# maelaubert/VulkanSift

Measured on AMD Instinct MI355X. Metric: SIFT detect+match frames/sec (640x480, ~2k kp), higher is better.
Workload: dtype f32

## Files before the change

### include/vksift_hip.h

```cpp
#ifndef VKSIFT_HIP_H
#define VKSIFT_HIP_H

#include <stddef.h>
#include <stdint.h>

#ifdef __cplusplus
extern "C"
{
#endif

#define VKSIFT_HIP_MAX_TAPS 20
#define VKSIFT_HIP_MATCH_CHUNKS 32
#define VKSIFT_HIP_MATCH_SMALL_NA 1536u
#define VKSIFT_HIP_MATCH_SMALL_NB 4096u
#define VKSIFT_HIP_MATCH_SCRATCH_U32(na, nb) (2u * (size_t)(na) + (size_t)(nb) + 72u + (size_t)(na) * 16u * VKSIFT_HIP_MATCH_CHUNKS)
#define VKSIFT_HIP_ABI_VERSION 6u
#define VKSIFT_HIP_GATHER_SLOTS 512u
#define VKSIFT_HIP_MATCH_SLOTS 256u
#define VKSIFT_HIP_MATCH_PK_NB 32768u
#define VKSIFT_HIP_MAX_ORI 18
#define VKSIFT_HIP_MAX_OCTAVE_SIDE 16383u

  typedef void *vksift_hip_stream;
  typedef void *vksift_hip_graph;
  typedef void *vksift_hip_event;

  int vksift_hip_init(void);
  uint32_t vksift_hip_abi_version(void);
  int vksift_hip_device_count(void);
  int vksift_hip_device_name(int idx, char *out256);
  int vksift_hip_set_device(int idx);
  size_t vksift_hip_device_free_mem(void);
  void *vksift_hip_malloc(size_t bytes);
  void vksift_hip_free(void *p);
  void *vksift_hip_host_malloc(size_t bytes);
  void vksift_hip_host_free(void *p);
  int vksift_hip_host_register(void *p, size_t bytes);
  int vksift_hip_host_unregister(void *p);
  int vksift_hip_is_pinned(const void *p);
  vksift_hip_stream vksift_hip_stream_create(void);
  void vksift_hip_stream_destroy(vksift_hip_stream s);
  int vksift_hip_stream_sync(vksift_hip_stream s);
  int vksift_hip_stream_busy(vksift_hip_stream s);
  vksift_hip_event vksift_hip_event_create(void);
  void vksift_hip_event_destroy(vksift_hip_event e);
  int vksift_hip_event_record(vksift_hip_event e, vksift_hip_stream s);
  int vksift_hip_event_sync(vksift_hip_event e);
  int vksift_hip_event_busy(vksift_hip_event e);
  float vksift_hip_event_elapsed_ms(vksift_hip_event a, vksift_hip_event b);
  int vksift_hip_stream_wait_event(vksift_hip_stream s, vksift_hip_event e);
  int vksift_hip_capture_begin(vksift_hip_stream s);
  int vksift_hip_capture_end(vksift_hip_stream s, vksift_hip_graph *out);
  int vksift_hip_graph_launch(vksift_hip_graph g, vksift_hip_stream s);
  void vksift_hip_graph_destroy(vksift_hip_graph g);
  int vksift_hip_memcpy_h2d(void *dst, const void *src, size_t n, vksift_hip_stream s);
  int vksift_hip_memcpy_d2h(void *dst, const void *src, size_t n, vksift_hip_stream s);
  int vksift_hip_memcpy_d2d(void *dst, const void *src, size_t n, vksift_hip_stream s);
  int vksift_hip_memcpy2d_d2h(void *dst, size_t dpitch, const void *src, size_t spitch, size_t width_bytes, size_t height, vksift_hip_stream s);
  int vksift_hip_post_words(uint32_t *host_mapped_dst, const uint32_t *src, size_t n_words, vksift_hip_stream s);
  int vksift_hip_memset(void *dst, int value, size_t n, vksift_hip_stream s);
  const char *vksift_hip_error_string(int err);
  void vksift_hip_range_push(const char *name);
  void vksift_hip_range_pop(void);

  enum
  {
    VKSIFT_TUNE_WG_TARGET = 0,
    VKSIFT_TUNE_WIDE_MASK = 1,
    VKSIFT_TUNE_MULTI_MAX = 2,
    VKSIFT_TUNE_REFINE_PTR = 3,
    VKSIFT_TUNE_SCAN_FORM = 4,
    VKSIFT_TUNE_PAIR_FORM = 5,
    VKSIFT_TUNE_PYR_GATE = 6,
    VKSIFT_TUNE_DENSE_ROWS = 7,
    VKSIFT_TUNE_SEED_WG = 8,
    VKSIFT_TUNE_SCAN_BAND = 9,
    VKSIFT_TUNE_TAIL_MULTI = 10,
    VKSIFT_TUNE_ZERO_COPY = 11,
    VKSIFT_TUNE_MIN_MARCH = 12,
    VKSIFT_TUNE_COUNT = 16
  };
  int vksift_hip_tune(int knob, int value);
  int vksift_hip_tune_get(int knob);


  typedef struct
  {
    float *base;
    uint32_t w, h;
    uint32_t pitch;
    uint64_t img_stride;
    uint32_t fp16;
    uint32_t reverse;
  } vksift_hip_Plane;

  int vksift_hip_input_blit(const uint8_t *src, uint32_t sw, uint32_t sh, uint64_t src_img_stride, vksift_hip_Plane dst, uint32_t batch,
                            vksift_hip_stream s);

  int vksift_hip_blur(vksift_hip_Plane src, vksift_hip_Plane dst, const float *taps, uint32_t ntaps, uint32_t batch, vksift_hip_stream s);

  int vksift_hip_blur_pair(vksift_hip_Plane src, vksift_hip_Plane dst1, vksift_hip_Plane dst2, const float *taps1, uint32_t ntaps1, const float *taps2,
                           uint32_t ntaps2, uint32_t batch, vksift_hip_stream s);

  int vksift_hip_blur_form(vksift_hip_Plane src, vksift_hip_Plane dst, uint32_t ntaps, uint32_t batch);

  int vksift_hip_blur_multi(const vksift_hip_Plane *src, const vksift_hip_Plane *dst, uint32_t n, const float *taps, uint32_t ntaps, uint32_t batch,
                            vksift_hip_stream s);

  int vksift_hip_blur_downsample(vksift_hip_Plane src, vksift_hip_Plane dst, vksift_hip_Plane next, const float *taps, uint32_t ntaps, uint32_t batch,
                                 vksift_hip_stream s);

  int vksift_hip_seed_upsampled(const uint8_t *src, uint32_t sw, uint32_t sh, uint64_t src_img_stride, vksift_hip_Plane dst, const float *taps, uint32_t ntaps,
                                uint32_t batch, vksift_hip_stream s);

  int vksift_hip_seed_direct(const uint8_t *src, uint32_t sw, uint32_t sh, uint64_t src_img_stride, vksift_hip_Plane dst, const float *taps, uint32_t ntaps,
                             uint32_t batch, vksift_hip_stream s);

  int vksift_hip_downsample(vksift_hip_Plane src, vksift_hip_Plane dst, uint32_t batch, vksift_hip_stream s);

  int vksift_hip_octave_chain(const vksift_hip_Plane *layers, uint32_t n_oct, uint32_t n_layers, uint32_t S, const float *taps, const uint32_t *ntaps,
                              uint32_t batch, vksift_hip_stream s);

  int vksift_hip_dog_plane(const float *lo, const float *hi, uint32_t w, uint32_t h, uint32_t pitch, uint32_t fp16, float *out_dense, vksift_hip_stream s);

  typedef struct
  {
    float *gauss;
    uint32_t fp16;
    uint32_t w, h, pitch;
    uint64_t plane_stride;
    uint64_t img_stride;
    uint32_t S;
    int32_t octave_idx;
    float seed_sigma;
    float dog_threshold;
    float edge_limit;
    uint8_t *feats;
    uint64_t feat_img_stride;
    uint32_t cap;
    uint32_t *found;
    uint32_t found_img_stride;
    uint64_t *seg_mask;
    uint32_t *seg_off;
    uint64_t seg_img_stride;
    uint32_t *cand_xy;
    uint32_t *cand_flag;
    uint32_t *cand_n;
    uint64_t cand_img_stride;
    uint32_t cand_cap;
    float *ori_ang;
    uint32_t *ori_cnt;
    uint64_t ori_img_stride;
    uint32_t max_ori;
    uint32_t use_vlfeat;
    const float *desc_fp_tab;
    uint32_t desc_fp_tab_len;
    uint32_t scan_reverse;
    uint32_t masks_cleared;
    uint32_t sec_index;
  } vksift_hip_OctaveJob;

  typedef struct
// ... 62 lines not shown
```

### vulkansift_amd/csrc/hip/extrema.hip

```cpp
#include <hip/hip_runtime.h>
#include <type_traits>
#include <stdint.h>
#include <stdlib.h>

#include "../detmath.h"
#include "multi.h"
#include "vksift_hip.h"

namespace
{

struct DogView
{
  const float *base;
  int w, h, pitch;
  size_t plane;
  int S;
  int fp16;
};

template <bool F16>
__device__ __forceinline__ float ld(const DogView &d, int s, int x, int y)
{
  if (s < 0 || s > d.S + 1)
    return 0.f;
  if (F16)
  {
    const _Float16 *p = (const _Float16 *)d.base + (size_t)s * d.plane + (size_t)y * d.pitch + x;
    return (float)(_Float16)((float)p[d.plane] - (float)p[0]);
  }
  const float *p = d.base + (size_t)s * d.plane + (size_t)y * d.pitch + x;
  return p[d.plane] - p[0];
}

struct KpRecord
{
  float x, y, scale_x, scale_y;
  uint32_t scale_idx;
  int32_t octave_idx;
  float sigma, orientation, intensity;
};

template <bool F16>
__device__ bool refine_texel(const DogView &d, int x, int y, int s, float dog_threshold, float edge_limit, float seed_sigma, int octave_idx, KpRecord *kp)
{
  const int W = d.w, H = d.h, S = d.S;
  float oX = 0.f, oY = 0.f, oS = 0.f, gX = 0.f, gY = 0.f, gS = 0.f;
  int rx = x, ry = y, rs = s;
  for (int step = 0; step < 5; step++)
  {
    float vc = ld<F16>(d, rs, rx, ry);
    float sp = ld<F16>(d, rs + 1, rx, ry), sm = ld<F16>(d, rs - 1, rx, ry);
    float xp = ld<F16>(d, rs, rx + 1, ry), xm = ld<F16>(d, rs, rx - 1, ry);
    float yp = ld<F16>(d, rs, rx, ry + 1), ym = ld<F16>(d, rs, rx, ry - 1);
    gS = 0.5f * (sp - sm);
    gX = 0.5f * (xp - xm);
    gY = 0.5f * (yp - ym);
    float h11 = sp + sm - 2.f * vc;
    float h22 = xp + xm - 2.f * vc;
    float h33 = yp + ym - 2.f * vc;
    float h12 = 0.25f * (ld<F16>(d, rs + 1, rx + 1, ry) - ld<F16>(d, rs + 1, rx - 1, ry) - ld<F16>(d, rs - 1, rx + 1, ry) + ld<F16>(d, rs - 1, rx - 1, ry));
    float h13 = 0.25f * (ld<F16>(d, rs + 1, rx, ry + 1) - ld<F16>(d, rs + 1, rx, ry - 1) - ld<F16>(d, rs - 1, rx, ry + 1) + ld<F16>(d, rs - 1, rx, ry - 1));
    float h23 = 0.25f * (ld<F16>(d, rs, rx + 1, ry + 1) - ld<F16>(d, rs, rx + 1, ry - 1) - ld<F16>(d, rs, rx - 1, ry + 1) + ld<F16>(d, rs, rx - 1, ry - 1));

    float det = h11 * ((h22 * h33) - (h23 * h23)) - h12 * ((h12 * h33) - (h13 * h23)) + h13 * ((h12 * h23) - (h13 * h22));
    if (det == 0.0f)
      return false;
    float i11 = ((h22 * h33) - (h23 * h23)) / det;
    float i12 = -1.f * ((h12 * h33) - (h13 * h23)) / det;
    float i13 = ((h12 * h23) - (h13 * h22)) / det;
    float i22 = ((h11 * h33) - (h13 * h13)) / det;
    float i23 = -1.f * ((h11 * h23) - (h13 * h12)) / det;
    float i33 = ((h11 * h22) - (h12 * h12)) / det;
    oS = -i11 * gS - i12 * gX - i13 * gY;
    oX = -i12 * gS - i22 * gX - i23 * gY;
    oY = -i13 * gS - i23 * gX - i33 * gY;

    if (fabsf(oX) < 0.6f && fabsf(oY) < 0.6f && fabsf(oS) < 0.6f)
      break;
    else if (step < 4)
    {
      rx += ((oX >= 0.6f && rx < (W - 2)) ? 1 : 0) + ((oX <= -0.6f && rx > 1) ? -1 : 0);
      ry += ((oY >= 0.6f && ry < (H - 2)) ? 1 : 0) + ((oY <= -0.6f && ry > 1) ? -1 : 0);
      rs += ((oS >= 0.6f && rs < (S + 1)) ? 1 : 0) + ((oS <= -0.6f && rs > 1) ? -1 : 0);
    }
  }
  float sx = (float)rx + oX, sy = (float)ry + oY, ss = (float)rs + oS;
  float vc = ld<F16>(d, rs, rx, ry);
  float nv = vc + 0.5f * (gX * oX + gY * oY + gS * oS);
  if (!(fabsf(nv) > dog_threshold && fabsf(oX) < 1.5f && fabsf(oY) < 1.5f && fabsf(oS) < 1.5f && sx >= 0 && sx < (float)W && sy >= 0 && sy < (float)H &&
        ss >= 0 && ss <= (float)(S + 1)))
    return false;
  float e11 = ld<F16>(d, rs, rx + 1, ry) + ld<F16>(d, rs, rx - 1, ry) - 2.f * vc;
  float e22 = ld<F16>(d, rs, rx, ry + 1) + ld<F16>(d, rs, rx, ry - 1) - 2.f * vc;
  float e12 = 0.25f * (ld<F16>(d, rs, rx + 1, ry + 1) - ld<F16>(d, rs, rx + 1, ry - 1) - ld<F16>(d, rs, rx - 1, ry + 1) + ld<F16>(d, rs, rx - 1, ry - 1));
  float edgeness = ((e11 + e22) * (e11 + e22)) / ((e11 * e22) - (e12 * e12));
  if (!((edgeness < edge_limit) && (edgeness >= 0)))
    return false;

  float scale_factor = octave_idx >= 0 ? dm_pow2i(octave_idx) : 1.f / dm_pow2i(-octave_idx);
  kp->scale_x = sx;
  kp->scale_y = sy;
  kp->scale_idx = (uint32_t)roundf(ss);
  kp->octave_idx = octave_idx;
  kp->sigma = seed_sigma * dm_exp2f(ss / (float)S) * scale_factor;
  kp->orientation = 0.f;
  kp->intensity = nv;
  kp->x = sx * scale_factor;
  kp->y = sy * scale_factor;
  return true;
}

template <bool F16>
__device__ bool refine_texel_buf(const __amdgpu_buffer_rsrc_t rsrc, int W, int H, int pitch, unsigned plane, int S, int x, int y, int s, float dog_threshold,
                                 float edge_limit, float seed_sigma, int octave_idx, KpRecord *kp)
{
  constexpr unsigned EB = F16 ? 2u : 4u;
  const int pitch_b = pitch * (int)EB;
  const unsigned plane_b = plane * EB;
  auto tex = [&](unsigned base, int row_off) -> float {
    if (F16)
      return (float)__builtin_bit_cast(_Float16, (unsigned short)__builtin_amdgcn_raw_buffer_load_b16(rsrc, base, row_off, 0));
    return __uint_as_float(__builtin_amdgcn_raw_buffer_load_b32(rsrc, base, row_off, 0));
  };
  auto dog = [&](float hi, float lo) -> float { return F16 ? (float)(_Float16)(hi - lo) : hi - lo; };
  float oX = 0.f, oY = 0.f, oS = 0.f, gX = 0.f, gY = 0.f, gS = 0.f;
  float vc = 0.f, xp = 0.f, xm = 0.f, yp = 0.f, ym = 0.f, h23 = 0.f;
  int rx = x, ry = y, rs = s;
  for (int step = 0; step < 5; step++)
  {
    const unsigned b0 = ((unsigned)rs * plane + (unsigned)(ry - 1) * (unsigned)pitch + (unsigned)(rx - 1)) * EB;
    const unsigned bm = b0 - plane_b, b1 = b0 + plane_b, b2 = b1 + plane_b;
    float g0[3][3], g1[3][3];
#pragma unroll
    for (int j = 0; j < 3; j++)
#pragma unroll
      for (int i = 0; i < 3; i++)
      {
        g0[j][i] = tex(b0 + (unsigned)i * EB, j * pitch_b);
        g1[j][i] = tex(b1 + (unsigned)i * EB, j * pitch_b);
      }
    const float gm_c = tex(bm + EB, pitch_b), gm_xm = tex(bm, pitch_b), gm_xp = tex(bm + 2u * EB, pitch_b), gm_ym = tex(bm + EB, 0), gm_yp = tex(bm + EB, 2 * pitch_b);
    const float g2_c = tex(b2 + EB, pitch_b), g2_xm = tex(b2, pitch_b), g2_xp = tex(b2 + 2u * EB, pitch_b), g2_ym = tex(b2 + EB, 0), g2_yp = tex(b2 + EB, 2 * pitch_b);
    const bool up = rs + 1 <= S + 1;
    const float sp = up ? dog(g2_c, g1[1][1]) : 0.f, sm = dog(g0[1][1], gm_c);
    const float p_xp = up ? dog(g2_xp, g1[1][2]) : 0.f, p_xm = up ? dog(g2_xm, g1[1][0]) : 0.f;
    const float p_yp = up ? dog(g2_yp, g1[2][1]) : 0.f, p_ym = up ? dog(g2_ym, g1[0][1]) : 0.f;
    const float m_xp = dog(g0[1][2], gm_xp), m_xm = dog(g0[1][0], gm_xm), m_yp = dog(g0[2][1], gm_yp), m_ym = dog(g0[0][1], gm_ym);
    float d0[3][3];
#pragma unroll
    for (int j = 0; j < 3; j++)
#pragma unroll
      for (int i = 0; i < 3; i++)
        d0[j][i] = dog(g1[j][i], g0[j][i]);
    vc = d0[1][1];
    xp = d0[1][2], xm = d0[1][0], yp = d0[2][1], ym = d0[0][1];
    gS = 0.5f * (sp - sm);
    gX = 0.5f * (xp - xm);
    gY = 0.5f * (yp - ym);
    float h11 = sp + sm - 2.f * vc;
    float h22 = xp + xm - 2.f * vc;
    float h33 = yp + ym - 2.f * vc;
    float h12 = 0.25f * (p_xp - p_xm - m_xp + m_xm);
    float h13 = 0.25f * (p_yp - p_ym - m_yp + m_ym);
    h23 = 0.25f * (d0[2][2] - d0[0][2] - d0[2][0] + d0[0][0]);

    float det = h11 * ((h22 * h33) - (h23 * h23)) - h12 * ((h12 * h33) - (h13 * h23)) + h13 * ((h12 * h23) - (h13 * h22));
    if (det == 0.0f)
      return false;
    float i11 = ((h22 * h33) - (h23 * h23)) / det;
    float i12 = -1.f * ((h12 * h33) - (h13 * h23)) / det;
    float i13 = ((h12 * h23) - (h13 * h22)) / det;
    float i22 = ((h11 * h33) - (h13 * h13)) / det;
    float i23 = -1.f * ((h11 * h23) - (h13 * h12)) / det;
    float i33 = ((h11 * h22) - (h12 * h12)) / det;
    oS = -i11 * gS - i12 * gX - i13 * gY;
    oX = -i12 * gS - i22 * gX - i23 * gY;
    oY = -i13 * gS - i23 * gX - i33 * gY;

    if (fabsf(oX) < 0.6f && fabsf(oY) < 0.6f && fabsf(oS) < 0.6f)
      break;
    else if (step < 4)
    {
      rx += ((oX >= 0.6f && rx < (W - 2)) ? 1 : 0) + ((oX <= -0.6f && rx > 1) ? -1 : 0);
      ry += ((oY >= 0.6f && ry < (H - 2)) ? 1 : 0) + ((oY <= -0.6f && ry > 1) ? -1 : 0);
      rs += ((oS >= 0.6f && rs < (S + 1)) ? 1 : 0) + ((oS <= -0.6f && rs > 1) ? -1 : 0);
    }
  }
  float sx = (float)rx + oX, sy = (float)ry + oY, ss = (float)rs + oS;
  float nv = vc + 0.5f * (gX * oX + gY * oY + gS * oS);
  if (!(fabsf(nv) > dog_threshold && fabsf(oX) < 1.5f && fabsf(oY) < 1.5f && fabsf(oS) < 1.5f && sx >= 0 && sx < (float)W && sy >= 0 && sy < (float)H &&
        ss >= 0 && ss <= (float)(S + 1)))
    return false;
  float e11 = xp + xm - 2.f * vc;
  float e22 = yp + ym - 2.f * vc;
  float e12 = h23;
  float edgeness = ((e11 + e22) * (e11 + e22)) / ((e11 * e22) - (e12 * e12));
  if (!((edgeness < edge_limit) && (edgeness >= 0)))
    return false;

  float scale_factor = octave_idx >= 0 ? dm_pow2i(octave_idx) : 1.f / dm_pow2i(-octave_idx);
  kp->scale_x = sx;
  kp->scale_y = sy;
  kp->scale_idx = (uint32_t)roundf(ss);
  kp->octave_idx = octave_idx;
  kp->sigma = seed_sigma * dm_exp2f(ss / (float)S) * scale_factor;
  kp->orientation = 0.f;
  kp->intensity = nv;
  kp->x = sx * scale_factor;
  kp->y = sy * scale_factor;
  return true;
}

struct ExtremaArgs
{
  const float *gauss;
  int fp16;
  int w, h, pitch;
  uint64_t plane_stride, img_stride;
  int S, octave_idx;
  float seed_sigma, dog_threshold, edge_limit;
  uint64_t *seg_mask;
  uint32_t *seg_off;
  uint64_t seg_img_stride;
  int nseg;
  uint8_t *feats;
  uint64_t feat_img_stride;
  uint32_t cap;
  uint32_t *found;
  uint32_t found_img_stride;
  uint32_t *cand_xy;
  uint32_t *cand_flag;
  uint32_t *cand_n;
  uint64_t cand_img_stride;
  uint32_t cand_cap;
  int band;
  uint32_t nsegs;
  uint32_t nchunks;
  int scan_rev;
};

__device__ __forceinline__ float wave_shr1(float v, float edge)
{
  return __builtin_bit_cast(float, __builtin_amdgcn_update_dpp(__builtin_bit_cast(int, edge), __builtin_bit_cast(int, v), 0x138, 0xf, 0xf, false));
}
__device__ __forceinline__ float wave_shl1(float v, float edge)
{
  return __builtin_bit_cast(float, __builtin_amdgcn_update_dpp(__builtin_bit_cast(int, edge), __builtin_bit_cast(int, v), 0x130, 0xf, 0xf, false));
}

__device__ __forceinline__ float fmax2(float a, float b)
{
  float r;
  asm("v_max_f32 %0, %1, %2" : "=v"(r) : "v"(a), "v"(b));
  return r;
}
__device__ __forceinline__ float fmin2(float a, float b)
{
  float r;
  asm("v_min_f32 %0, %1, %2" : "=v"(r) : "v"(a), "v"(b));
  return r;
}
__device__ __forceinline__ float fmax3(float a, float b, float c)
{
  float r;
  asm("v_max3_f32 %0, %1, %2, %3" : "=v"(r) : "v"(a), "v"(b), "v"(c));
  return r;
}
__device__ __forceinline__ float fmin3(float a, float b, float c)
{
  float r;
  asm("v_min3_f32 %0, %1, %2, %3" : "=v"(r) : "v"(a), "v"(b), "v"(c));
  return r;
}

__device__ __forceinline__ unsigned long long spread32(unsigned long long x)
{
  x &= 0xFFFFFFFFull;
  x = (x | (x << 16)) & 0x0000FFFF0000FFFFull;
  x = (x | (x << 8)) & 0x00FF00FF00FF00FFull;
  x = (x | (x << 4)) & 0x0F0F0F0F0F0F0F0Full;
  x = (x | (x << 2)) & 0x3333333333333333ull;
  x = (x | (x << 1)) & 0x5555555555555555ull;
  return x;
}

typedef unsigned u32x2_t __attribute__((ext_vector_type(2)));
constexpr unsigned EXT_OOB = 0x80000000u;

template <int S, int NSLOT, bool F16>
__global__ void __launch_bounds__(256, 4) k_extrema_lean(Multi<ExtremaArgs> m, int strip_major)
{
  const VBlock vb = vblock(m);
// ... 192 lines not shown
  uint32_t *__restrict__ chunk_tot = a.cand_flag;
  const uint64_t chunk_img_stride = a.cand_img_stride;
  const uint32_t n = a.nsegs;
  const int lane = threadIdx.x & 63, wave = threadIdx.x >> 6;
  const uint32_t i0 = vb.x * SEG_CHUNK + 4u * threadIdx.x;
  uint32_t p[4];
#pragma unroll
  for (int k = 0; k < 4; k++)
    p[k] = i0 + k < n ? (uint32_t)__popcll(mask[i0 + k]) : 0u;
  const uint32_t tsum = p[0] + p[1] + p[2] + p[3];
  uint32_t incl = tsum;
#pragma unroll
  for (int dlt = 1; dlt < 64; dlt <<= 1)
  {
    uint32_t t = __shfl_up(incl, dlt, 64);
    if (lane >= dlt)
      incl += t;
  }
  if (lane == 63)
    wave_tot[wave] = incl;
  __syncthreads();
  uint32_t wave_base = 0, total = 0;
  for (int wv = 0; wv < 16; wv++)
  {
    if (wv < wave)
      wave_base += wave_tot[wv];
    total += wave_tot[wv];
  }
  uint32_t run = wave_base + incl - tsum;
#pragma unroll
  for (int k = 0; k < 4; k++)
  {
    if (i0 + k < n)
      off[i0 + k] = run;
    run += p[k];
  }
  if (threadIdx.x == 0)
    chunk_tot[(size_t)b * chunk_img_stride + vb.x] = total;
}


__global__ void __launch_bounds__(256) k_cand_list(Multi<ExtremaArgs> mu)
{
  const VBlock vb = vblock(mu);
  const ExtremaArgs &a = mu.oct[vb.o];
  const uint32_t seg = vb.x * 256 + threadIdx.x;
  const int b = (int)vb.y;
  const uint32_t *chunk_tot = a.cand_flag + (size_t)b * a.cand_img_stride;
  if (vb.x == 0 && threadIdx.x == 0)
  {
    uint32_t total = 0;
    for (uint32_t c = 0; c < a.nchunks; c++)
      total += chunk_tot[c];
    a.cand_n[b] = total;
    if (total == 0)
      a.found[(size_t)b * a.found_img_stride] = 0;
  }
  unsigned long long m = seg < a.nsegs ? a.seg_mask[seg + (size_t)b * a.seg_img_stride] : 0ull;
  if (__ballot(m != 0ull) == 0ull)
    return;
  uint32_t base = 0;
  for (uint32_t c = threadIdx.x & 63u, nc = (vb.x * 256u) / SEG_CHUNK; c < nc; c += 64u)
    base += chunk_tot[c];
#pragma unroll
  for (int dlt = 32; dlt >= 1; dlt >>= 1)
    base += __shfl_xor(base, dlt, 64);
  if (m == 0ull)
    return;
  uint32_t pos = a.seg_off[seg + (size_t)b * a.seg_img_stride] + base;
  const uint32_t segx = seg % (uint32_t)a.nseg;
  const uint32_t yy = (seg / (uint32_t)a.nseg) % (uint32_t)a.h;
  const uint32_t sz = seg / ((uint32_t)a.nseg * (uint32_t)a.h);
  uint32_t *out = a.cand_xy + (size_t)b * a.cand_img_stride;
  while (m)
  {
    const int bit = __ffsll((long long)m) - 1;
    m &= m - 1;
    if (pos < a.cand_cap)
      out[pos] = (segx * 64u + (uint32_t)bit) | (yy << 14) | ((sz + 1u) << 28);
    pos++;
  }
}

template <bool F16, bool BUF>
__global__ void __launch_bounds__(256) k_refine_flags(Multi<ExtremaArgs> m)
{
  __shared__ uint32_t s_cnt[4];
  const VBlock vb = vblock(m);
  const ExtremaArgs &a = m.oct[vb.o];
  const int b = (int)vb.x;
  uint32_t n = a.cand_n[b];
  n = n < a.cand_cap ? n : a.cand_cap;
  const uint32_t nch = (n + 255u) / 256u;
  DogView d{(const float *)((const uint8_t *)a.gauss + (size_t)b * a.img_stride * (a.fp16 ? 2u : 4u)), a.w, a.h, a.pitch, (size_t)a.plane_stride, a.S, a.fp16};
  const __amdgpu_buffer_rsrc_t rsrc =
      __builtin_amdgcn_make_buffer_rsrc((void *)d.base, 0, (int)((unsigned)(a.S + 3) * (unsigned)a.plane_stride * (F16 ? 2u : 4u)), 0x00020000);
  const uint32_t *xy = a.cand_xy + (size_t)b * a.cand_img_stride;
  uint32_t *flag = a.cand_flag + (size_t)b * a.cand_img_stride;
  uint32_t *chunk_sum = a.seg_off + (size_t)b * a.seg_img_stride;
  for (uint32_t chunk = vb.y; chunk < nch; chunk += vb.gy)
  {
    const uint32_t i = chunk * 256u + threadIdx.x;
    bool ok = false;
    if (i < n)
    {
      const uint32_t c = xy[i];
      KpRecord kp;
      const int cx = (int)(c & 0x3fffu), cy = (int)((c >> 14) & 0x3fffu), cs = (int)(c >> 28);
      ok = BUF ? refine_texel_buf<F16>(rsrc, a.w, a.h, a.pitch, (unsigned)a.plane_stride, a.S, cx, cy, cs, a.dog_threshold, a.edge_limit, a.seed_sigma, a.octave_idx, &kp)
               : refine_texel<F16>(d, cx, cy, cs, a.dog_threshold, a.edge_limit, a.seed_sigma, a.octave_idx, &kp);
      flag[i] = ok ? 1u : 0u;
    }
    const unsigned long long bal = __ballot(ok);
    if ((threadIdx.x & 63) == 0)
      s_cnt[threadIdx.x >> 6] = (uint32_t)__popcll(bal);
    __syncthreads();
    if (threadIdx.x == 0)
      chunk_sum[chunk] = s_cnt[0] + s_cnt[1] + s_cnt[2] + s_cnt[3];
    __syncthreads();
  }
}

template <bool F16, bool BUF>
__global__ void __launch_bounds__(256) k_cand_emit(Multi<ExtremaArgs> m)
{
  __shared__ uint32_t s_cnt[4];
  __shared__ uint32_t s_red[4];
  __shared__ uint32_t s_list[256];
  const VBlock vb = vblock(m);
  const ExtremaArgs &a = m.oct[vb.o];
  const int b = (int)vb.x;
  const int lane = threadIdx.x & 63, wave = threadIdx.x >> 6;
  uint32_t n = a.cand_n[b];
  n = n < a.cand_cap ? n : a.cand_cap;
  const uint32_t nch = (n + 255u) / 256u;
  DogView d{(const float *)((const uint8_t *)a.gauss + (size_t)b * a.img_stride * (a.fp16 ? 2u : 4u)), a.w, a.h, a.pitch, (size_t)a.plane_stride, a.S, a.fp16};
  const __amdgpu_buffer_rsrc_t rsrc =
      __builtin_amdgcn_make_buffer_rsrc((void *)d.base, 0, (int)((unsigned)(a.S + 3) * (unsigned)a.plane_stride * (F16 ? 2u : 4u)), 0x00020000);
  const uint32_t *xy = a.cand_xy + (size_t)b * a.cand_img_stride;
  const uint32_t *flag = a.cand_flag + (size_t)b * a.cand_img_stride;
  const uint32_t *chunk_sum = a.seg_off + (size_t)b * a.seg_img_stride;
  for (uint32_t chunk = vb.y; chunk < nch; chunk += vb.gy)
  {
    uint32_t part = 0;
    for (uint32_t c = threadIdx.x; c < chunk; c += 256u)
      part += chunk_sum[c];
#pragma unroll
    for (int dlt = 32; dlt >= 1; dlt >>= 1)
      part += __shfl_xor(part, dlt, 64);
    const uint32_t i = chunk * 256u + threadIdx.x;
    const bool v = i < n && flag[i] != 0u;
    const unsigned long long bal = __ballot(v);
    if (lane == 0)
      s_cnt[wave] = (uint32_t)__popcll(bal), s_red[wave] = part;
    __syncthreads();
    const uint32_t cbase = s_red[0] + s_red[1] + s_red[2] + s_red[3];
    uint32_t rank = (uint32_t)__popcll(bal & ((1ull << lane) - 1ull));
    for (int wv = 0; wv < wave; wv++)
      rank += s_cnt[wv];
    const uint32_t total = s_cnt[0] + s_cnt[1] + s_cnt[2] + s_cnt[3];
    if (v)
      s_list[rank] = xy[i];
    __syncthreads();
    const uint32_t idx = cbase + threadIdx.x;
    if (chunk + 1u == nch && threadIdx.x == 0)
      a.found[(size_t)b * a.found_img_stride] = cbase + total;
    if (threadIdx.x < total && idx < a.cap)
    {
      const uint32_t c = s_list[threadIdx.x];
      KpRecord kp;
      const int cx = (int)(c & 0x3fffu), cy = (int)((c >> 14) & 0x3fffu), cs = (int)(c >> 28);
      if (BUF)
        refine_texel_buf<F16>(rsrc, a.w, a.h, a.pitch, (unsigned)a.plane_stride, a.S, cx, cy, cs, a.dog_threshold, a.edge_limit, a.seed_sigma, a.octave_idx, &kp);
      else
        refine_texel<F16>(d, cx, cy, cs, a.dog_threshold, a.edge_limit, a.seed_sigma, a.octave_idx, &kp);
      uint32_t *rec = (uint32_t *)(a.feats + (size_t)b * a.feat_img_stride + (size_t)idx * 164);
      rec[0] = __float_as_uint(kp.x);
      rec[1] = __float_as_uint(kp.y);
      rec[2] = __float_as_uint(kp.scale_x);
      rec[3] = __float_as_uint(kp.scale_y);
      rec[4] = kp.scale_idx;
      rec[5] = (uint32_t)kp.octave_idx;
      rec[6] = __float_as_uint(kp.sigma);
      rec[7] = __float_as_uint(kp.orientation);
      rec[8] = __float_as_uint(kp.intensity);
    }
    __syncthreads();
  }
}

}

static int make_extrema_args(const vksift_hip_OctaveJob *job, ExtremaArgs *out)
{
  if (job->w > VKSIFT_HIP_MAX_OCTAVE_SIDE || job->h > VKSIFT_HIP_MAX_OCTAVE_SIDE || job->S > 14u)
    return (int)hipErrorInvalidValue;
  ExtremaArgs a;
  a.gauss = job->gauss;
  a.fp16 = (int)job->fp16;
  a.w = (int)job->w, a.h = (int)job->h, a.pitch = (int)job->pitch;
  a.plane_stride = job->plane_stride, a.img_stride = job->img_stride;
  a.S = (int)job->S, a.octave_idx = job->octave_idx;
  a.seed_sigma = job->seed_sigma, a.dog_threshold = job->dog_threshold, a.edge_limit = job->edge_limit;
  a.seg_mask = job->seg_mask, a.seg_off = job->seg_off, a.seg_img_stride = job->seg_img_stride;
  a.nseg = (int)((job->w + 63) / 64);
  a.feats = job->feats, a.feat_img_stride = job->feat_img_stride, a.cap = job->cap;
  a.found = job->found, a.found_img_stride = job->found_img_stride;
  a.cand_xy = job->cand_xy, a.cand_flag = job->cand_flag, a.cand_n = job->cand_n;
  a.cand_img_stride = job->cand_img_stride, a.cand_cap = job->cand_cap;
  a.scan_rev = (int)job->scan_reverse;
  a.band = job->h > 256u ? 48 : 16;
  if (vksift_hip_tune_get(VKSIFT_TUNE_SCAN_BAND) > 0 && job->h > 256u)
    a.band = vksift_hip_tune_get(VKSIFT_TUNE_SCAN_BAND);
  a.nsegs = job->S * job->h * (uint32_t)a.nseg;
  a.nchunks = (a.nsegs + SEG_CHUNK - 1u) / SEG_CHUNK;
  if (job->seg_img_stride != a.nsegs || a.nchunks > a.cand_cap)
    return (int)hipErrorInvalidValue;
  *out = a;
  return 0;
}

static int clear_masks(const ExtremaArgs *args, uint32_t n, uint32_t batch, hipStream_t hs)
{
  for (uint32_t i = 0; i < n;)
  {
    uint32_t j = i + 1;
    size_t bytes = sizeof(uint64_t) * (size_t)args[i].nsegs * batch;
    while (j < n && (const uint8_t *)args[j].seg_mask == (const uint8_t *)args[i].seg_mask + bytes)
      bytes += sizeof(uint64_t) * (size_t)args[j].nsegs * batch, j++;
    const hipError_t me = hipMemsetAsync(args[i].seg_mask, 0, bytes, hs);
    if (me != hipSuccess)
      return (int)me;
    i = j;
  }
  return 0;
}

static int extract_run(const vksift_hip_OctaveJob *jobs, uint32_t n, uint32_t batch, hipStream_t hs, hipEvent_t scan_done)
{
  ExtremaArgs args[MULTI_MAX];
  for (uint32_t i = 0; i < n; i++)
  {
    const int e = make_extrema_args(&jobs[i], &args[i]);
    if (e)
      return e;
  }
  const bool f16 = args[0].fp16 != 0;
  const int S = args[0].S;
  {
    uint64_t waves = 0;
    for (uint32_t i = 0; i < n; i++)
      waves += (uint64_t)batch * ((args[i].w + 127) / 128) * ((args[i].h + args[i].band - 1) / args[i].band);
    if (waves < 2048u && vksift_hip_tune_get(VKSIFT_TUNE_SCAN_BAND) <= 0)
      for (uint32_t i = 0; i < n; i++)
        args[i].band = 16;
  }

  bool cleared = true;
  for (uint32_t i = 0; i < n; i++)
    cleared = cleared && jobs[i].masks_cleared != 0;
  if (!cleared)
  {
    const int me = clear_masks(args, n, batch, hs);
    if (me)
      return me;
  }
  const int sm = 3;
  for (uint32_t i = 0; i < n; i++)
    if ((uint64_t)jobs[i].pitch * jobs[i].h * (f16 ? 2u : 4u) >= 0x80000000ull)
      return (int)hipErrorInvalidValue;

#define VKSIFT_MULTI(M, GX, GY, GZ)                              \
  Multi<ExtremaArgs> M;                                           \
  M.n = 0;                                                        \
  for (uint32_t i = 0; i < n; i++)                                \
  {                                                               \
    const ExtremaArgs &a = args[i];                               \
    (void)a;                                                      \
    if (!multi_add(M, args[i], (GX), (GY), (GZ)))                 \
      return (int)hipErrorInvalidValue;                           \
  }
  {
    VKSIFT_MULTI(ms, (uint32_t)(a.nseg + 1) / 2u, ((a.h + a.band - 1) / a.band + 3u) / 4u, batch)
    const dim3 sgrid(ms.start[ms.n]);
    switch (S)
    {
#define VKSIFT_CASE(N)                                                                \
  case N:                                                                             \
    if (f16)                                                                          \
      hipLaunchKernelGGL((k_extrema_lean<N, 5, true>), sgrid, dim3(256), 0, hs, ms, sm);  \
    else                                                                              \
      hipLaunchKernelGGL((k_extrema_lean<N, 4, false>), sgrid, dim3(256), 0, hs, ms, sm); \
    break;
      VKSIFT_CASE(1) VKSIFT_CASE(2) VKSIFT_CASE(3) VKSIFT_CASE(4) VKSIFT_CASE(5) VKSIFT_CASE(6) VKSIFT_CASE(7) VKSIFT_CASE(8) VKSIFT_CASE(9)
      VKSIFT_CASE(10) VKSIFT_CASE(11) VKSIFT_CASE(12) VKSIFT_CASE(13)
#undef VKSIFT_CASE
    default:
      return (int)hipErrorInvalidValue;
    }
  }
  if (scan_done)
    (void)hipEventRecord(scan_done, hs);
  {
    VKSIFT_MULTI(m2, a.nchunks, batch, 1u)
    hipLaunchKernelGGL(k_segment_scan, dim3(m2.start[m2.n]), dim3(1024), 0, hs, m2);
  }
  {
    VKSIFT_MULTI(m3, (a.nsegs + 255u) / 256u, batch, 1u)
    hipLaunchKernelGGL(k_cand_list, dim3(m3.start[m3.n]), dim3(256), 0, hs, m3);
  }
  const uint32_t rcap = 65536u / batch < 16u ? 16u : (65536u / batch > 512u ? 512u : 65536u / batch);
#define VKSIFT_REFINE_CHUNKS(a) (((uint64_t)(a).S * (uint32_t)(a).w * (uint32_t)(a).h / 4u + 64u + 255u) / 256u)
  VKSIFT_MULTI(mr, batch, VKSIFT_REFINE_CHUNKS(a) > rcap ? rcap : (uint32_t)VKSIFT_REFINE_CHUNKS(a), 1u)
#undef VKSIFT_REFINE_CHUNKS
  const dim3 rgrid(mr.start[mr.n]);
  bool buf = vksift_hip_tune_get(VKSIFT_TUNE_REFINE_PTR) == 0;
  for (uint32_t i = 0; i < n; i++)
    buf = buf && (uint64_t)(args[i].S + 3) * args[i].plane_stride * (f16 ? 2u : 4u) < 0x7FFF0000ull;
  if (f16 && buf)
    hipLaunchKernelGGL((k_refine_flags<true, true>), rgrid, dim3(256), 0, hs, mr);
  else if (f16)
    hipLaunchKernelGGL((k_refine_flags<true, false>), rgrid, dim3(256), 0, hs, mr);
  else if (buf)
    hipLaunchKernelGGL((k_refine_flags<false, true>), rgrid, dim3(256), 0, hs, mr);
  else
    hipLaunchKernelGGL((k_refine_flags<false, false>), rgrid, dim3(256), 0, hs, mr);
  if (f16 && buf)
    hipLaunchKernelGGL((k_cand_emit<true, true>), rgrid, dim3(256), 0, hs, mr);
  else if (f16)
    hipLaunchKernelGGL((k_cand_emit<true, false>), rgrid, dim3(256), 0, hs, mr);
  else if (buf)
    hipLaunchKernelGGL((k_cand_emit<false, true>), rgrid, dim3(256), 0, hs, mr);
  else
    hipLaunchKernelGGL((k_cand_emit<false, false>), rgrid, dim3(256), 0, hs, mr);
#undef VKSIFT_MULTI
  return (int)hipGetLastError();
}

extern "C" int vksift_hip_extract_keypoints_multi(const vksift_hip_OctaveJob *jobs, uint32_t n_jobs, uint32_t batch, vksift_hip_stream s,
                                                  vksift_hip_event scan_done)
{
  if (n_jobs == 0 || batch == 0)
    return 0;
  for (uint32_t i0 = 0; i0 < n_jobs;)
  {
    uint32_t i1 = i0 + 1;
    while (i1 < n_jobs && i1 - i0 < multi_run_max() && jobs[i1].S == jobs[i0].S && jobs[i1].fp16 == jobs[i0].fp16)
      i1++;
    const int e = extract_run(jobs + i0, i1 - i0, batch, (hipStream_t)s, i1 == n_jobs ? (hipEvent_t)scan_done : nullptr);
    if (e)
      return e;
    i0 = i1;
  }
  return 0;
}

extern "C" int vksift_hip_clear_segment_masks(const vksift_hip_OctaveJob *jobs, uint32_t n_jobs, uint32_t batch, vksift_hip_stream s)
{
  if (n_jobs == 0 || batch == 0)
    return 0;
  if (n_jobs > 16)
    return (int)hipErrorInvalidValue;
  ExtremaArgs args[16];
  for (uint32_t i = 0; i < n_jobs; i++)
  {
    const int e = make_extrema_args(&jobs[i], &args[i]);
    if (e)
      return e;
  }
  return clear_masks(args, n_jobs, batch, (hipStream_t)s);
}

extern "C" int vksift_hip_extract_keypoints(const vksift_hip_OctaveJob *job, uint32_t batch, vksift_hip_stream s, vksift_hip_event scan_done)
{
  return vksift_hip_extract_keypoints_multi(job, 1, batch, s, scan_done);
}
```

Before: 25140.

## Refine keypoint candidates once and stash results in candidate buffers

Replaces the refine-flags plus emit pair, which ran the subpixel refinement twice per accepted candidate, with a single refinement pass. That pass writes the refined core values (position, scale, response) compactly into the candidate xy/flag buffers for chunks with few accepted points, and a move kernel then turns them into full records. Chunks with more accepted points than the cap fall back to flagging and re-refining. The old path stays selectable through a new tune knob, and the change adds per-chunk stash layout logic and a different grid cap for the move kernel.

New measurement: 25210 (median of 6 runs). No clear change (+0.3%).

```diff
diff --git a/include/vksift_hip.h b/include/vksift_hip.h
--- a/include/vksift_hip.h
+++ b/include/vksift_hip.h
@@ -78,6 +78,7 @@
     VKSIFT_TUNE_TAIL_MULTI = 10,
     VKSIFT_TUNE_ZERO_COPY = 11,
     VKSIFT_TUNE_MIN_MARCH = 12,
+    VKSIFT_TUNE_EXTRACT_FORM = 13,
     VKSIFT_TUNE_COUNT = 16
   };
   int vksift_hip_tune(int knob, int value);
diff --git a/vulkansift_amd/csrc/hip/extrema.hip b/vulkansift_amd/csrc/hip/extrema.hip
--- a/vulkansift_amd/csrc/hip/extrema.hip
+++ b/vulkansift_amd/csrc/hip/extrema.hip
@@ -41,8 +41,27 @@
   float sigma, orientation, intensity;
 };
 
+struct KpCore
+{
+  float sx, sy, ss, nv;
+};
+
+__device__ __forceinline__ void finish_record(const KpCore &c, int S, float seed_sigma, int octave_idx, KpRecord *kp)
+{
+  float scale_factor = octave_idx >= 0 ? dm_pow2i(octave_idx) : 1.f / dm_pow2i(-octave_idx);
+  kp->scale_x = c.sx;
+  kp->scale_y = c.sy;
+  kp->scale_idx = (uint32_t)roundf(c.ss);
+  kp->octave_idx = octave_idx;
+  kp->sigma = seed_sigma * dm_exp2f(c.ss / (float)S) * scale_factor;
+  kp->orientation = 0.f;
+  kp->intensity = c.nv;
+  kp->x = c.sx * scale_factor;
+  kp->y = c.sy * scale_factor;
+}
+
 template <bool F16>
-__device__ bool refine_texel(const DogView &d, int x, int y, int s, float dog_threshold, float edge_limit, float seed_sigma, int octave_idx, KpRecord *kp)
+__device__ bool refine_texel(const DogView &d, int x, int y, int s, float dog_threshold, float edge_limit, KpCore *kp)
 {
   const int W = d.w, H = d.h, S = d.S;
   float oX = 0.f, oY = 0.f, oS = 0.f, gX = 0.f, gY = 0.f, gS = 0.f;
@@ -98,22 +117,13 @@
   if (!((edgeness < edge_limit) && (edgeness >= 0)))
     return false;
 
-  float scale_factor = octave_idx >= 0 ? dm_pow2i(octave_idx) : 1.f / dm_pow2i(-octave_idx);
-  kp->scale_x = sx;
-  kp->scale_y = sy;
-  kp->scale_idx = (uint32_t)roundf(ss);
-  kp->octave_idx = octave_idx;
-  kp->sigma = seed_sigma * dm_exp2f(ss / (float)S) * scale_factor;
-  kp->orientation = 0.f;
-  kp->intensity = nv;
-  kp->x = sx * scale_factor;
-  kp->y = sy * scale_factor;
+  kp->sx = sx, kp->sy = sy, kp->ss = ss, kp->nv = nv;
   return true;
 }
 
 template <bool F16>
 __device__ bool refine_texel_buf(const __amdgpu_buffer_rsrc_t rsrc, int W, int H, int pitch, unsigned plane, int S, int x, int y, int s, float dog_threshold,
-                                 float edge_limit, float seed_sigma, int octave_idx, KpRecord *kp)
+                                 float edge_limit, KpCore *kp)
 {
   constexpr unsigned EB = F16 ? 2u : 4u;
   const int pitch_b = pitch * (int)EB;
@@ -199,16 +209,7 @@
   if (!((edgeness < edge_limit) && (edgeness >= 0)))
     return false;
 
-  float scale_factor = octave_idx >= 0 ? dm_pow2i(octave_idx) : 1.f / dm_pow2i(-octave_idx);
-  kp->scale_x = sx;
-  kp->scale_y = sy;
-  kp->scale_idx = (uint32_t)roundf(ss);
-  kp->octave_idx = octave_idx;
-  kp->sigma = seed_sigma * dm_exp2f(ss / (float)S) * scale_factor;
-  kp->orientation = 0.f;
-  kp->intensity = nv;
-  kp->x = sx * scale_factor;
-  kp->y = sy * scale_factor;
+  kp->sx = sx, kp->sy = sy, kp->ss = ss, kp->nv = nv;
   return true;
 }
 
@@ -567,6 +568,22 @@
   }
 }
 
+__device__ __forceinline__ void store_record(const ExtremaArgs &a, int b, uint32_t idx, const KpCore &kc)
+{
+  KpRecord kp;
+  finish_record(kc, a.S, a.seed_sigma, a.octave_idx, &kp);
+  uint32_t *rec = (uint32_t *)(a.feats + (size_t)b * a.feat_img_stride + (size_t)idx * 164);
+  rec[0] = __float_as_uint(kp.x);
+  rec[1] = __float_as_uint(kp.y);
+  rec[2] = __float_as_uint(kp.scale_x);
+  rec[3] = __float_as_uint(kp.scale_y);
+  rec[4] = kp.scale_idx;
+  rec[5] = (uint32_t)kp.octave_idx;
+  rec[6] = __float_as_uint(kp.sigma);
+  rec[7] = __float_as_uint(kp.orientation);
+  rec[8] = __float_as_uint(kp.intensity);
+}
+
 template <bool F16, bool BUF>
 __global__ void __launch_bounds__(256) k_refine_flags(Multi<ExtremaArgs> m)
 {
@@ -590,10 +607,10 @@
     if (i < n)
     {
       const uint32_t c = xy[i];
-      KpRecord kp;
+      KpCore kc;
       const int cx = (int)(c & 0x3fffu), cy = (int)((c >> 14) & 0x3fffu), cs = (int)(c >> 28);
-      ok = BUF ? refine_texel_buf<F16>(rsrc, a.w, a.h, a.pitch, (unsigned)a.plane_stride, a.S, cx, cy, cs, a.dog_threshold, a.edge_limit, a.seed_sigma, a.octave_idx, &kp)
-               : refine_texel<F16>(d, cx, cy, cs, a.dog_threshold, a.edge_limit, a.seed_sigma, a.octave_idx, &kp);
+      ok = BUF ? refine_texel_buf<F16>(rsrc, a.w, a.h, a.pitch, (unsigned)a.plane_stride, a.S, cx, cy, cs, a.dog_threshold, a.edge_limit, &kc)
+               : refine_texel<F16>(d, cx, cy, cs, a.dog_threshold, a.edge_limit, &kc);
       flag[i] = ok ? 1u : 0u;
     }
     const unsigned long long bal = __ballot(ok);
@@ -653,22 +670,146 @@
     if (threadIdx.x < total && idx < a.cap)
     {
       const uint32_t c = s_list[threadIdx.x];
-      KpRecord kp;
+      KpCore kc;
       const int cx = (int)(c & 0x3fffu), cy = (int)((c >> 14) & 0x3fffu), cs = (int)(c >> 28);
       if (BUF)
-        refine_texel_buf<F16>(rsrc, a.w, a.h, a.pitch, (unsigned)a.plane_stride, a.S, cx, cy, cs, a.dog_threshold, a.edge_limit, a.seed_sigma, a.octave_idx, &kp);
+        refine_texel_buf<F16>(rsrc, a.w, a.h, a.pitch, (unsigned)a.plane_stride, a.S, cx, cy, cs, a.dog_threshold, a.edge_limit, &kc);
       else
-        refine_texel<F16>(d, cx, cy, cs, a.dog_threshold, a.edge_limit, a.seed_sigma, a.octave_idx, &kp);
-      uint32_t *rec = (uint32_t *)(a.feats + (size_t)b * a.feat_img_stride + (size_t)idx * 164);
-      rec[0] = __float_as_uint(kp.x);
-      rec[1] = __float_as_uint(kp.y);
-      rec[2] = __float_as_uint(kp.scale_x);
-      rec[3] = __float_as_uint(kp.scale_y);
-      rec[4] = kp.scale_idx;
-      rec[5] = (uint32_t)kp.octave_idx;
-      rec[6] = __float_as_uint(kp.sigma);
-      rec[7] = __float_as_uint(kp.orientation);
-      rec[8] = __float_as_uint(kp.intensity);
+        refine_texel<F16>(d, cx, cy, cs, a.dog_threshold, a.edge_limit, &kc);
+      store_record(a, b, idx, kc);
+    }
+    __syncthreads();
+  }
+}
+
+constexpr uint32_t REC_CHUNK_CAP = 128;
+
+__device__ __forceinline__ bool chunk_is_compact(uint32_t chunk, uint32_t accepted, uint32_t rec_cap, uint32_t cand_cap)
+{
+  return accepted <= rec_cap && (uint64_t)chunk * 256u + 256u <= (uint64_t)cand_cap;
+}
+
+template <bool F16, bool BUF>
+__global__ void __launch_bounds__(256) k_refine_once(Multi<ExtremaArgs> m, uint32_t rec_cap)
+{
+  __shared__ uint32_t s_cnt[4];
+  const VBlock vb = vblock(m);
+  const ExtremaArgs &a = m.oct[vb.o];
+  const int b = (int)vb.x;
+  const int lane = threadIdx.x & 63, wave = threadIdx.x >> 6;
+  uint32_t n = a.cand_n[b];
+  n = n < a.cand_cap ? n : a.cand_cap;
+  const uint32_t nch = (n + 255u) / 256u;
+  DogView d{(const float *)((const uint8_t *)a.gauss + (size_t)b * a.img_stride * (a.fp16 ? 2u : 4u)), a.w, a.h, a.pitch, (size_t)a.plane_stride, a.S, a.fp16};
+  const __amdgpu_buffer_rsrc_t rsrc =
+      __builtin_amdgcn_make_buffer_rsrc((void *)d.base, 0, (int)((unsigned)(a.S + 3) * (unsigned)a.plane_stride * (F16 ? 2u : 4u)), 0x00020000);
+  uint32_t *xy = a.cand_xy + (size_t)b * a.cand_img_stride;
+  uint32_t *flag = a.cand_flag + (size_t)b * a.cand_img_stride;
+  uint32_t *chunk_sum = a.seg_off + (size_t)b * a.seg_img_stride;
+  for (uint32_t chunk = vb.y; chunk < nch; chunk += vb.gy)
+  {
+    const uint32_t i = chunk * 256u + threadIdx.x;
+    bool ok = false;
+    KpCore kc{0.f, 0.f, 0.f, 0.f};
+    if (i < n)
+    {
+      const uint32_t c = xy[i];
+      const int cx = (int)(c & 0x3fffu), cy = (int)((c >> 14) & 0x3fffu), cs = (int)(c >> 28);
+      ok = BUF ? refine_texel_buf<F16>(rsrc, a.w, a.h, a.pitch, (unsigned)a.plane_stride, a.S, cx, cy, cs, a.dog_threshold, a.edge_limit, &kc)
+               : refine_texel<F16>(d, cx, cy, cs, a.dog_threshold, a.edge_limit, &kc);
+    }
+    const unsigned long long bal = __ballot(ok);
+    if (lane == 0)
+      s_cnt[wave] = (uint32_t)__popcll(bal);
+    __syncthreads();
+    uint32_t rank = (uint32_t)__popcll(bal & ((1ull << lane) - 1ull));
+    for (int wv = 0; wv < wave; wv++)
+      rank += s_cnt[wv];
+    const uint32_t total = s_cnt[0] + s_cnt[1] + s_cnt[2] + s_cnt[3];
+    if (chunk_is_compact(chunk, total, rec_cap, a.cand_cap))
+    {
+      if (ok)
+      {
+        uint32_t *r0 = xy + (size_t)chunk * 256u + rank, *r1 = flag + (size_t)chunk * 256u + rank;
+        r0[0] = __float_as_uint(kc.sx), r0[REC_CHUNK_CAP] = __float_as_uint(kc.sy);
+        r1[0] = __float_as_uint(kc.ss), r1[REC_CHUNK_CAP] = __float_as_uint(kc.nv);
+      }
+    }
+    else if (i < n)
+      flag[i] = ok ? 1u : 0u;
+    if (threadIdx.x == 0)
+      chunk_sum[chunk] = total;
+    __syncthreads();
+  }
+}
+
+template <bool F16, bool BUF>
+__global__ void __launch_bounds__(256) k_cand_move(Multi<ExtremaArgs> m, uint32_t rec_cap)
+{
+  __shared__ uint32_t s_cnt[4];
+  __shared__ uint32_t s_red[4];
+  __shared__ uint32_t s_list[256];
+  const VBlock vb = vblock(m);
+  const ExtremaArgs &a = m.oct[vb.o];
+  const int b = (int)vb.x;
+  const int lane = threadIdx.x & 63, wave = threadIdx.x >> 6;
+  uint32_t n = a.cand_n[b];
+  n = n < a.cand_cap ? n : a.cand_cap;
+  const uint32_t nch = (n + 255u) / 256u;
+  const uint32_t *xy = a.cand_xy + (size_t)b * a.cand_img_stride;
+  const uint32_t *flag = a.cand_flag + (size_t)b * a.cand_img_stride;
+  const uint32_t *chunk_sum = a.seg_off + (size_t)b * a.seg_img_stride;
+  for (uint32_t chunk = vb.y; chunk < nch; chunk += vb.gy)
+  {
+    uint32_t part = 0;
+    for (uint32_t c = threadIdx.x; c < chunk; c += 256u)
+      part += chunk_sum[c];
+#pragma unroll
+    for (int dlt = 32; dlt >= 1; dlt >>= 1)
+      part += __shfl_xor(part, dlt, 64);
+    const uint32_t total = chunk_sum[chunk];
+    const bool compact = chunk_is_compact(chunk, total, rec_cap, a.cand_cap);
+    const uint32_t i = chunk * 256u + threadIdx.x;
+    const bool v = !compact && i < n && flag[i] != 0u;
+    const unsigned long long bal = __ballot(v);
+    if (lane == 0)
+      s_cnt[wave] = (uint32_t)__popcll(bal), s_red[wave] = part;
+    __syncthreads();
+    const uint32_t cbase = s_red[0] + s_red[1] + s_red[2] + s_red[3];
+    const uint32_t idx = cbase + threadIdx.x;
+    if (chunk + 1u == nch && threadIdx.x == 0)
+      a.found[(size_t)b * a.found_img_stride] = cbase + total;
+    if (compact)
+    {
+      if (threadIdx.x < total && idx < a.cap)
+      {
+        const uint32_t *r0 = xy + (size_t)chunk * 256u + threadIdx.x, *r1 = flag + (size_t)chunk * 256u + threadIdx.x;
+        const KpCore kc{__uint_as_float(r0[0]), __uint_as_float(r0[REC_CHUNK_CAP]), __uint_as_float(r1[0]), __uint_as_float(r1[REC_CHUNK_CAP])};
+        store_record(a, b, idx, kc);
+      }
+    }
+    else
+    {
+      uint32_t rank = (uint32_t)__popcll(bal & ((1ull << lane) - 1ull));
+      for (int wv = 0; wv < wave; wv++)
+        rank += s_cnt[wv];
+      if (v)
+        s_list[rank] = xy[i];
+      __syncthreads();
+      if (threadIdx.x < total && idx < a.cap)
+      {
+        DogView d{(const float *)((const uint8_t *)a.gauss + (size_t)b * a.img_stride * (a.fp16 ? 2u : 4u)), a.w, a.h, a.pitch, (size_t)a.plane_stride, a.S, a.fp16};
+        const __amdgpu_buffer_rsrc_t rsrc =
+            __builtin_amdgcn_make_buffer_rsrc((void *)d.base, 0, (int)((unsigned)(a.S + 3) * (unsigned)a.plane_stride * (F16 ? 2u : 4u)), 0x00020000);
+        const uint32_t c = s_list[threadIdx.x];
+        KpCore kc;
+        const int cx = (int)(c & 0x3fffu), cy = (int)((c >> 14) & 0x3fffu), cs = (int)(c >> 28);
+        if (BUF)
+          refine_texel_buf<F16>(rsrc, a.w, a.h, a.pitch, (unsigned)a.plane_stride, a.S, cx, cy, cs, a.dog_threshold, a.edge_limit, &kc);
+        else
+          refine_texel<F16>(d, cx, cy, cs, a.dog_threshold, a.edge_limit, &kc);
+        store_record(a, b, idx, kc);
+      }
     }
     __syncthreads();
   }
@@ -802,22 +943,33 @@
   bool buf = vksift_hip_tune_get(VKSIFT_TUNE_REFINE_PTR) == 0;
   for (uint32_t i = 0; i < n; i++)
     buf = buf && (uint64_t)(args[i].S + 3) * args[i].plane_stride * (f16 ? 2u : 4u) < 0x7FFF0000ull;
-  if (f16 && buf)
-    hipLaunchKernelGGL((k_refine_flags<true, true>), rgrid, dim3(256), 0, hs, mr);
-  else if (f16)
-    hipLaunchKernelGGL((k_refine_flags<true, false>), rgrid, dim3(256), 0, hs, mr);
-  else if (buf)
-    hipLaunchKernelGGL((k_refine_flags<false, true>), rgrid, dim3(256), 0, hs, mr);
+  const int form = vksift_hip_tune_get(VKSIFT_TUNE_EXTRACT_FORM);
+  const uint32_t rec_cap = form >= 2 && (uint32_t)form < REC_CHUNK_CAP ? (uint32_t)form : REC_CHUNK_CAP;
+#define VKSIFT_LAUNCH2(K, GRID, ...)                                                       \
+  do                                                                                  \
+  {                                                                                   \
+    if (f16 && buf)                                                                   \
+      hipLaunchKernelGGL((K<true, true>), GRID, dim3(256), 0, hs, __VA_ARGS__);      \
+    else if (f16)                                                                     \
+      hipLaunchKernelGGL((K<true, false>), GRID, dim3(256), 0, hs, __VA_ARGS__);     \
+    else if (buf)                                                                     \
+      hipLaunchKernelGGL((K<false, true>), GRID, dim3(256), 0, hs, __VA_ARGS__);     \
+    else                                                                              \
+      hipLaunchKernelGGL((K<false, false>), GRID, dim3(256), 0, hs, __VA_ARGS__);    \
+  } while (0)
+  if (form == 1)
+  {
+    VKSIFT_LAUNCH2(k_refine_flags, rgrid, mr);
+    VKSIFT_LAUNCH2(k_cand_emit, rgrid, mr);
+  }
   else
-    hipLaunchKernelGGL((k_refine_flags<false, false>), rgrid, dim3(256), 0, hs, mr);
-  if (f16 && buf)
-    hipLaunchKernelGGL((k_cand_emit<true, true>), rgrid, dim3(256), 0, hs, mr);
-  else if (f16)
-    hipLaunchKernelGGL((k_cand_emit<true, false>), rgrid, dim3(256), 0, hs, mr);
-  else if (buf)
-    hipLaunchKernelGGL((k_cand_emit<false, true>), rgrid, dim3(256), 0, hs, mr);
-  else
-    hipLaunchKernelGGL((k_cand_emit<false, false>), rgrid, dim3(256), 0, hs, mr);
+  {
+    VKSIFT_LAUNCH2(k_refine_once, rgrid, mr, rec_cap);
+    const uint32_t mcap = 8192u / batch < 16u ? 16u : (8192u / batch > 512u ? 512u : 8192u / batch);
+    VKSIFT_MULTI(mv, batch, mr.gy[i] > mcap ? mcap : mr.gy[i], 1u)
+    VKSIFT_LAUNCH2(k_cand_move, dim3(mv.start[mv.n]), mv, rec_cap);
+  }
+#undef VKSIFT_LAUNCH2
 #undef VKSIFT_MULTI
   return (int)hipGetLastError();
 }
```
